# NAIST-Archlab/vsim

Hardware: AMD Instinct MI355X
Metric: decode tokens/sec GPT-J-6B Q4_0 @1 GPU; achieved HBM GB/s vs peak (higher is better)
Workload: dtype f32 (Q4_0 x Q4_0 operands); 1 GPU; gpt-j-6B Q4_0 decode, 874 timed tokens after a 5-token prompt + 5 warm-up tokens, batch 1; mode=exact, n_ctx=980, parallelism=single, graph=True

## Files before the change

include/vsim_hip.h:

```cpp
#ifndef VSIM_HIP_H
#define VSIM_HIP_H

#include <stddef.h>
#include <stdint.h>

#include "ggml_abi.h"

#ifdef __cplusplus
extern "C" {
#endif

#define VSIM_OK 0
#define VSIM_EINVAL (-1)
#define VSIM_EHIP (-2)
#define VSIM_ENOMEM (-3)
#define VSIM_EFILE (-4)
#define VSIM_ENODEV (-5)
#define VSIM_ESPIN (-6)

#define VSIM_MODE_EXACT 0
#define VSIM_MODE_FAST 1

#define VSIM_ARCH_GPTNEOX 0
#define VSIM_ARCH_GPTJ 1
// ... 47 lines not shown
int vsim_batch_set_gemm(int enable);
int vsim_op_q4_gemm_fast_rows(const void *w, int M, int K, const void *xq, int n, const float *bias, float *y,
                              void *stream);
int vsim_batch_set_fast_gemm(int enable);
typedef struct {
  const float *q, *k, *v;
  float *const *kc;
  float *const *vc;
  const int32_t *n_past;
  const double *cs;
  const float *alibi;
  int32_t B, d, H, n_rot, style, n_ctx, kqv_nth;
  float scale;
  float *out;
  void *oq;
  float *oxd;
} vsim_attn_batch_args;
int vsim_op_attn_decode_batch(const vsim_attn_batch_args *a, void *stream);
int vsim_op_q4_expand_f16(const void *w, int M, int K, void *w16, void *stream);
int vsim_op_gemm_f16(const void *w16, int M, int K, const void *x16, int n, const float *bias, float *y,
                     void *stream);
int vsim_op_act_quant_f16(const float *x, int K, int n, const float *bias, int gelu, void *x16, void *stream);
int vsim_op_gemm_f16_gelu_q(const void *w16, int M, int K, const void *x16, int n, const float *bias, void *q16,
                            void *stream);
int vsim_op_gemm_f16_rope(const void *w16, int M, int K, const void *x16, int n, const float *bias, float *y,
                          const double *cs, int d, int n_rot, int p0, void *stream);
int vsim_op_gemm_f16_join(const void *w16, int M, int K, const void *x16, int n, const float *bias, float *res,
                          const float *res_a, void *stream);
int vsim_op_gemm_q4_256(const void *w, int M, int K, const void *x16, int n, const float *bias, float *y, void *q16,
                        const double *cs, int d, int n_rot, int p0, int join, const float *res_a, void *stream);
int vsim_op_get_rows(const void *w, int K, int V, const int32_t *rows, int n, float *y, void *stream);
int vsim_op_norm(const float *x, float *y, int k, int rows, const float *w, const float *b, void *stream);
int vsim_norm_fallbacks(unsigned out[2]);
int vsim_spin_timeouts(unsigned *out);
int vsim_op_gelu(const float *x, float *y, int n, void *stream);
int vsim_op_argmax(const float *x, int n, int32_t *out, void *stream);
#define VSIM_TOPK_MAX 64
#define VSIM_WINDOW_MAX 1024
int vsim_op_topk(const float *x, int n, const int32_t *win, int nw, double scale, double repeat_penalty, int k,
                 double *val, int32_t *id, void *stream);
int vsim_op_logprob(const float *x, int V, int R, const int32_t *target, double *logprob, int32_t *argmax,
                    void *stream);
int vsim_op_attn_softmax(float *p, int nc, int nr, int nz, int n_past, float scale, void *stream);
int vsim_op_rope(int style, float *x, int d, int H, int T, int n_past, int n_dims, int mode, void *stream);
int vsim_op_kq(const float *K, int ldk, const float *Q, int ldq, int d, int H, int nk, int n, float *kq,
               void *stream);
int vsim_op_kqv(const float *V, int ldv, const float *S, int d, int H, int nk, int n, float *out, void *stream);
int vsim_op_kq_causal(const float *K, int ldk, const float *Q, int ldq, int d, int H, int nk, int n, int n_past,
                      float *kq, void *stream);
int vsim_op_kqv_causal(const float *V, int ldv, const float *S, int d, int H, int nk, int n, int n_past, float *out,
                       void *stream);
int vsim_op_attn_prefill(const float *Q, const float *kc, const float *vc, int d, int H, int N, int n_past,
                         float scale, float *out, void *stream);
int vsim_op_attn_prefill_q16(const float *Q, const float *kc, const float *vc, int d, int H, int N, int n_past,
                             float scale, void *out16, void *stream);
int vsim_gemm_set_streamk(int enable);
int vsim_op_gemm_q4_256_pair(const void *w0, const void *w1, int M, int K, const void *x16, int n, float *y0, float *y1,
                             const double *cs, int d, int n_rot, int p0, void *stream);
int vsim_gemm_set_qk_pair(int mode);
int vsim_gemm_set_tile_order(int cols);
int vsim_op_norm_f16q(const float *x, int k, int rows, const float *w, const float *b, void *x16, void *stream);
#define VSIM_FAST_PAD 65536
enum { VSIM_FE_STORE = 0, VSIM_FE_GELU_Q = 1, VSIM_FE_ROPE_Q = 2, VSIM_FE_ROPE_K = 3, VSIM_FE_V = 4 };
typedef struct {
  const void *w;
  int32_t rows, k;
// ... 116 lines not shown
```

vsim_amd/csrc/capi.cpp:

```cpp
#include <hip/hip_runtime.h>

#include <cstdio>
#include <cstdlib>
#include <cstring>
#include <mutex>
#include <unordered_map>
#include <map>
#include <vector>

#include "common.hpp"
#include "fast.hpp"
#include "graph.hpp"
#include "../../include/vsim_hip.h"

namespace vsim {
int tables_host(uint16_t *exp_f16, uint16_t *gelu_f16);
}

using namespace vsim;

#define RC(x)                \
  do {                       \
    int rc_ = (x);           \
    if (rc_) return rc_;     \
// ... 117 lines not shown
  if (!w16 || !x16 || !res) { set_error("gemm_f16_join: null argument"); return VSIM_EINVAL; }
  G2Epi e;
  e.res = res;
  e.res_a = res_a;
  return launch_gemm_f16_256(w16, M, K, x16, n, bias, res, (hipStream_t)stream, nullptr, &e);
}
int vsim_op_gemm_q4_256(const void *w, int M, int K, const void *x16, int n, const float *bias, float *y, void *q16,
                        const double *cs, int d, int n_rot, int p0, int join, const float *res_a, void *stream) {
  if (!w || !x16 || (!q16 && !y) || M <= 0 || K <= 0 || K % QK || p0 < 0) {
    set_error("gemm_q4_256: bad argument");
    return VSIM_EINVAL;
  }
  if ((q16 != nullptr) + (cs != nullptr) + (join != 0) > 1) {
    set_error("gemm_q4_256: one epilogue at a time (q16, cs or join)");
    return VSIM_EINVAL;
  }
  G2Epi e;
  if (cs) {
    e.cs = (const double2 *)cs;
    e.d = d;
    e.n_rot = n_rot;
    e.p0 = p0;
  } else if (join) {
    e.res = y;
    e.res_a = res_a;
  }
  return launch_gemm_q4_256(w4_view(w, M, K), x16, n, bias, q16 ? nullptr : y, (hipStream_t)stream, q16,
                            cs || join ? &e : nullptr);
}
int vsim_op_get_rows(const void *w, int K, int V, const int32_t *rows, int n, float *y, void *stream) {
  return launch_get_rows(w, K, V, rows, n, y, (hipStream_t)stream);
}
int vsim_norm_fallbacks(unsigned out[2]) { return vsim::norm_stats(out); }
int vsim_spin_timeouts(unsigned *out) { return vsim::spin_timeouts(out); }

int vsim_op_norm(const float *x, float *y, int k, int rows, const float *w, const float *b, void *stream) {
  return launch_norm(x, y, k, rows, w, b, (hipStream_t)stream);
}
int vsim_op_gelu(const float *x, float *y, int n, void *stream) {
  return launch_gelu(x, y, n, nullptr, 1, (hipStream_t)stream);
}
int vsim_op_argmax(const float *x, int n, int32_t *out, void *stream) {
  static std::mutex mu;
  static std::map<std::pair<int, void *>, unsigned long long *> wss;
  int dev = 0;
  VSIM_HIP(hipGetDevice(&dev));
  unsigned long long *ws = nullptr;
  {
    std::lock_guard<std::mutex> lk(mu);
    unsigned long long *&w = wss[{dev, stream}];
    if (!w) {
      VSIM_HIP(hipMalloc((void **)&w, 2 * sizeof(unsigned long long)));
      VSIM_HIP(hipMemset(w, 0, 2 * sizeof(unsigned long long)));
    }
    ws = w;
  }
  return launch_argmax(x, n, (int *)out, ws, (hipStream_t)stream);
}
int vsim_op_topk(const float *x, int n, const int32_t *win, int nw, double scale, double repeat_penalty, int k,
                 double *val, int32_t *id, void *stream) {
  static std::mutex mu;
  static std::map<std::pair<int, void *>, void *> wss;
  int dev = 0;
  VSIM_HIP(hipGetDevice(&dev));
  void *ws = nullptr;
  {
// ... 471 lines not shown
```

vsim_amd/csrc/common.hpp:

```cpp
#pragma once

#include <hip/hip_runtime.h>
#include <stdint.h>

#include <map>
#include <string>

#include "../../include/vsim_hip.h"

namespace vsim {

constexpr int QK = 32;
constexpr int QBYTES = 20;

constexpr int T32 = 32;

typedef float f32x4 __attribute__((ext_vector_type(4)));
typedef unsigned int u32x4 __attribute__((ext_vector_type(4)));

struct W4 {
  const uint8_t *qs;
  const float *d;
  int rows, k, tiles;
  __host__ __device__ int nb() const { return k / QK; }
// ... 32 lines not shown
struct GemvBatch {
  GemvJob j[4];
  int nj;
};

struct LnQuantJob {
  const float *x;
  const float *w, *b;
  uint8_t *qs;
  float *d;
  float *xd;
  const float *ja, *jab, *jf, *jfb;
  float *jout;
  unsigned *ep;
};

struct TailLn {
  const float *x;
  const float *ab, *fb;
  float *jout;
  const float *w1, *b1;
  uint8_t *q1;
  float *d1, *xd1;
  const float *w2, *b2;
  uint8_t *q2;
  float *d2, *xd2;
  unsigned long long *og, *jg;
  uint4 *rec;
  const unsigned *ep;
  unsigned *stats;
  int il;
};
constexpr int LNT_MAX_TILES = 256;

struct AttnJob {
  const float *q, *k, *v;
  float *kc, *vc;
  const int *npast;
  const double2 *cs;
  const uint16_t *etab;
  int d, H, n_rot, style;
  int n_ctx;
  int nsplit;
  int kqv_nth;
  float scale;
  const float *alibi;
  uint8_t *oq_qs;
  float *oq_d, *oxd;
  float *out;
};

constexpr int ATT_VTF = 8192;
__host__ __device__ constexpr int attn_lds_floats(int d, int n_ctx) {
  return ((2 * d + n_ctx + 3) & ~3) + 2 * ATT_VTF;
}

int launch_ln_quant(const LnQuantJob &j0, const LnQuantJob *j1, int n, hipStream_t s);
int launch_residual_join(const float *x, const float *a, const float *ab, const float *f, const float *fb, float *out,
                         int n, hipStream_t s);
int launch_gemv_epi(const GemvBatch &B, int mode, hipStream_t s);
int launch_attn_decode(const AttnJob &A, int n_ctx, hipStream_t s);
struct AttnRows {
  float *const *kc, *const *vc;
  size_t loff;
  const int *npast;
};
// ... 77 lines not shown
}

__device__ __forceinline__ float wave_sum_f(float v) {
  return dpp::lane63(dpp::reduce(v, 0.0f, [](float a, float b) { return a + b; }));
}
__device__ __forceinline__ double wave_sum_d(double v) {
  return dpp::lane63(dpp::reduce(v, 0.0, [](double a, double b) { return a + b; }));
}
__device__ __forceinline__ float wave_max_f(float v) {
  return dpp::lane63(dpp::reduce(v, -INFINITY, [](float a, float b) { return fmaxf(a, b); }));
}
__device__ __forceinline__ int wave_min_i(int v) {
  return dpp::lane63(dpp::reduce(v, 0x7FFFFFFF, [](int a, int b) { return min(a, b); }));
}

void set_error(const std::string &msg);
int hip_fail(hipError_t e, const char *what);
#define VSIM_HIP(call)                                          \
  do {                                                          \
    hipError_t e_ = (call);                                     \
    if (e_ != hipSuccess) return ::vsim::hip_fail(e_, #call);   \
  } while (0)

struct DevTables {
  const uint16_t *exp_f16;
  const uint16_t *gelu_f16;
};
int tables_get(DevTables *t);
unsigned *dev_stats();
unsigned *spin_error_counter();
unsigned *set_spin_error_target(unsigned *p);
void add_model_spin_timeouts(unsigned n);
int norm_stats(unsigned *out2);
int spin_timeouts(unsigned *out);

int launch_q4_repack(const void *aos, void *soa, int rows, int k, hipStream_t s);
int launch_q4_unpack(const void *soa, void *aos, int rows, int k, hipStream_t s);
int launch_q4_quantize(const float *x, int k, int n, void *xq, float *xd, hipStream_t s);
int launch_quantize_w(const void *x, int src_type, int rows, int k, void *w, int w_rows, int row0, void *aos,
                      uint64_t *hist, hipStream_t s);
int launch_q4_gemv(const void *w, int M, int K, const void *xq, const float *xd, int n, const float *bias,
                   float *y, int mode, hipStream_t s);
int launch_gemv_batch(const GemvBatch &B, int mode, hipStream_t s);
int launch_gemm_exact(const W4 &W, const float *xd, int n, const float *bias, float *y, hipStream_t s);
int launch_gemm_exact_rows(const W4 &W, const float *xd, int n, const float *bias, float *y, hipStream_t s);
int launch_gemm_fast_rows(const W4 &W, const void *xq, int n, const float *bias, float *y, hipStream_t s);
int batch_set_fast_gemm(int enable);
bool batch_fast_gemm_rows(int n);
int launch_act_repack(const void *aos, void *xq, int n, int k, hipStream_t s);
int launch_act_unpack(const void *xq, void *aos, int n, int k, hipStream_t s);
int launch_q4_dequant(const void *xq, int rows, int k, float *y, hipStream_t s);
int launch_get_rows(const void *w, int K, int V, const int32_t *rows, int n, float *y, hipStream_t s);
int launch_norm(const float *x, float *y, int k, int rows, const float *w, const float *b, hipStream_t s);
int launch_norm_f16q(const float *x, void *x16, int k, int rows, const float *w, const float *b, hipStream_t s);
int launch_argmax(const float *x, int n, int *out, unsigned long long *ws, hipStream_t s);
struct TopkParams {
  double scale, penalty;
  int32_t k, nw;
  int32_t win[VSIM_WINDOW_MAX];
};
struct TopkOut {
  double val[VSIM_TOPK_MAX];
  int32_t id[VSIM_TOPK_MAX];
};
constexpr int TOPK_MAX_WG = 64;
constexpr size_t TOPK_WS_BYTES = 256 + (size_t)TOPK_MAX_WG * 64 * (sizeof(unsigned long long) + sizeof(uint32_t));
// ... 79 lines not shown
```

vsim_amd/csrc/gemv_chain.hip:

```cpp
#include <cstdlib>
#include <cstring>

#ifdef VSIM_NB_STAMPS
namespace vsim {
__device__ unsigned long long g_nb_stamps[2048][32];
}
#define ATT_STAMP(i) \
  if (threadIdx.x == 0) g_nb_stamps[1536 + blockIdx.x][4 + (i)] = __builtin_amdgcn_s_memrealtime()
#endif
#include "attn.hpp"
#include "kern.hpp"
#include "../../include/vsim_hip.h"

namespace vsim {

typedef const __attribute__((address_space(4))) float sfloat;
typedef const __attribute__((address_space(1))) u32x4 gu32x4;
typedef const __attribute__((address_space(1))) float gfloat;

__device__ __forceinline__ void producer_barrier() { asm volatile("s_barrier" ::: "memory"); }


constexpr int waitcnt_vm(int n) { return 0x0F70 | (n & 15) | ((n >> 4) << 14); }
constexpr int c2_waves(int npw, bool fill) {
// ... 211 lines not shown
#define NB_ADDS4P(acc, a, o)                                                                                     \
  asm volatile(NB_PAIR(1, 2, 3, 4) NB_PAIR(5, 6, 7, 8) NB_PAIR(9, 10, 11, 12) NB_PAIR(13, 14, 15, 16)              \
               : "+v"(acc)                                                                                       \
               : "v"(a[o].x), "v"(a[o].y), "v"(a[o].z), "v"(a[o].w), "v"(a[o + 1].x), "v"(a[o + 1].y),           \
                 "v"(a[o + 1].z), "v"(a[o + 1].w), "v"(a[o + 2].x), "v"(a[o + 2].y), "v"(a[o + 2].z),            \
                 "v"(a[o + 2].w), "v"(a[o + 3].x), "v"(a[o + 3].y), "v"(a[o + 3].z), "v"(a[o + 3].w)             \
               : "memory")
#ifdef VSIM_NB_STAMPS
#define NBS(...) __VA_ARGS__
#else
#define NBS(...)
#endif
#ifndef NB_RING_N
#define NB_RING_N 4
#endif
constexpr int NB_RING = NB_RING_N;
constexpr unsigned NB_SPIN_MAX = 1u << 24;
template <class S>
struct NbLds {
  float P[NB_RING][32 * S::LD];
  uint4 RQ[S::DEPTH][S::NPW][64];
  float RD[S::DEPTH][S::NPW][64];
  float RX[S::DEPTH][S::NPW][64];
  unsigned ready[NB_RING];
  unsigned cons;
};

__device__ __forceinline__ unsigned lds_load(const unsigned *p) {
  return __hip_atomic_load(p, __ATOMIC_RELAXED, __HIP_MEMORY_SCOPE_WORKGROUP);
}

constexpr unsigned LNT_SPIN_MAX = 1u << 22;
typedef __attribute__((address_space(1))) unsigned long long gu64;
__device__ __forceinline__ unsigned lnt_tag(const TailLn &N) { return (*N.ep << 8) | (unsigned)(N.il + 1); }
__device__ __forceinline__ void st_granule(unsigned long long *p, float v, unsigned tag) {
  const unsigned long long g = (unsigned long long)__float_as_uint(v) | ((unsigned long long)tag << 32);
  __hip_atomic_store((gu64 *)p, g, __ATOMIC_RELAXED, __HIP_MEMORY_SCOPE_AGENT);
}
__device__ __forceinline__ unsigned long long ld_granule(const unsigned long long *p) {
  return __hip_atomic_load((const gu64 *)p, __ATOMIC_RELAXED, __HIP_MEMORY_SCOPE_AGENT);
}
__device__ __forceinline__ void st16_sc1(uint4 *p, u32x4 v) {
  asm volatile("global_store_dwordx4 %0, %1, off sc1" ::"v"(p), "v"(v) : "memory");
}
__device__ __forceinline__ double dbl_of(unsigned lo, unsigned hi) {
  return __longlong_as_double((long long)(((unsigned long long)hi << 32) | lo));
}
__device__ __forceinline__ void lnt_spin(unsigned &spins, unsigned *err, int lane) {
  __builtin_amdgcn_s_sleep(1);
  if (++spins == LNT_SPIN_MAX && err && lane == 0) __hip_atomic_fetch_add(err, 1u, __ATOMIC_RELAXED, __HIP_MEMORY_SCOPE_AGENT);
}

__device__ __forceinline__ void lnt_oproj(const TailLn &N, int row, int rows, float acc, int lane) {
  if (lane < 32 && row < rows) st_granule(N.og + row, acc, lnt_tag(N));
  NBS(if (lane == 0) g_nb_stamps[1536 + blockIdx.x][8] = __builtin_amdgcn_s_memrealtime();)
}

struct LntPre {
  unsigned long long g;
  float x, ab, fb, w, b;
};
__device__ __forceinline__ LntPre lnt_prefetch(const TailLn &N, int t) {
  const int lane = threadIdx.x & 63, i = t * T32 + (lane & 31);
  const bool hi = lane >= 32, mine = !hi || N.w2 != nullptr;
  LntPre p;
  p.g = ld_granule(N.og + i);
  p.x = N.x[i];
  p.ab = N.ab ? N.ab[i] : 0.0f;
  p.fb = N.fb ? N.fb[i] : 0.0f;
  p.w = mine ? (hi ? N.w2 : N.w1)[i] : 0.0f;
  p.b = mine ? (hi ? N.b2 : N.b1)[i] : 0.0f;
  return p;
}
__device__ __forceinline__ double half_sum_d(double v) {
  v = v + dpp::mov<dpp::QP_XOR1, 0xF>(v, 0.0);
  v = v + dpp::mov<dpp::QP_XOR2, 0xF>(v, 0.0);
  v = v + dpp::mov<dpp::HALF_MIRROR, 0xF>(v, 0.0);
  v = v + dpp::mov<dpp::MIRROR, 0xF>(v, 0.0);
  const long long b = __double_as_longlong(v);
  const int lo = __builtin_amdgcn_ds_swizzle((int)(b & 0xFFFFFFFF), 0x401F), hi = __builtin_amdgcn_ds_swizzle((int)(b >> 32), 0x401F);
  return v + __longlong_as_double(((long long)hi << 32) | (unsigned)lo);
}
__device__ __forceinline__ int half_min_i(int v) {
  v = min(v, dpp::mov<dpp::QP_XOR1, 0xF>(v, 0x7FFFFFFF));
  v = min(v, dpp::mov<dpp::QP_XOR2, 0xF>(v, 0x7FFFFFFF));
  v = min(v, dpp::mov<dpp::HALF_MIRROR, 0xF>(v, 0x7FFFFFFF));
  v = min(v, dpp::mov<dpp::MIRROR, 0xF>(v, 0x7FFFFFFF));
  return min(v, __builtin_amdgcn_ds_swizzle(v, 0x401F));
}

__device__ __forceinline__ void lnt_owner(const TailLn &N, int t, int ntile, float acc, const LntPre &pre,
                                          float *scr, unsigned *err) {
  const int lane = threadIdx.x & 63, i = t * T32 + (lane & 31), n = ntile * T32;
  const unsigned tag = lnt_tag(N);
  NBS(unsigned long long *ls = g_nb_stamps[1536 + blockIdx.x] + 8;
      if (lane == 0) ls[0] = __builtin_amdgcn_s_memrealtime();)
  const bool hi = lane >= 32, two = N.w2 != nullptr, mine = !hi || two;
  const float xv = pre.x, abv = pre.ab, fbv = pre.fb, wv = pre.w, bv = pre.b;
  unsigned spins = 0;
  unsigned long long ga = pre.g;
  while (!__all((unsigned)(ga >> 32) == tag) && spins < LNT_SPIN_MAX) {
    lnt_spin(spins, err, lane);
    ga = ld_granule(N.og + i);
  }
  NBS(if (lane == 0) {
    ls[1] = __builtin_amdgcn_s_memrealtime();
    ls[5] = spins;
  })
  const float a = N.ab ? __uint_as_float((unsigned)ga) + abv : __uint_as_float((unsigned)ga);
  const float ff = N.fb ? acc + fbv : acc;
  const float v = xv + (a + ff);
  {
    const double s = half_sum_d((double)v), sa = half_sum_d((double)fabsf(v));
    const double q = half_sum_d((double)v * (double)v);
    const int um = half_min_i(ulp_exp(v));
    if (lane == 0) {
      float au = (float)sa;
      if ((double)au < sa) au = __uint_as_float(__float_as_uint(au) + 1u);
      const unsigned long long sb = (unsigned long long)__double_as_longlong(s), qb = (unsigned long long)__double_as_longlong(q);
      st16_sc1(N.rec + 2 * t, u32x4{(unsigned)sb, (unsigned)(sb >> 32), (unsigned)um, tag});
      st16_sc1(N.rec + 2 * t + 1, u32x4{(unsigned)qb, (unsigned)(qb >> 32), __float_as_uint(au), tag});
    }
  }
  if (lane < 32) {
    N.jout[i] = v;
    st_granule(N.jg + i, v, tag);
  }
  NBS(if (lane == 0) ls[2] = __builtin_amdgcn_s_memrealtime();)
  const int ng = 2 * ntile;
  double S = 0.0, Q = 0.0, A = 0.0;
  int U = 1 << 30;
  spins = 0;
  for (;;) {
    u32x4 g[8];
    const uint4 *p[8];
#pragma unroll
    for (int k = 0; k < 8; ++k) p[k] = N.rec + min(lane + 64 * k, ng - 1);
    asm volatile(
        "global_load_dwordx4 %0, %8, off sc1\n\t"
        "global_load_dwordx4 %1, %9, off sc1\n\t"
        "global_load_dwordx4 %2, %10, off sc1\n\t"
        "global_load_dwordx4 %3, %11, off sc1\n\t"
        "global_load_dwordx4 %4, %12, off sc1\n\t"
        "global_load_dwordx4 %5, %13, off sc1\n\t"
        "global_load_dwordx4 %6, %14, off sc1\n\t"
        "global_load_dwordx4 %7, %15, off sc1\n\t"
        "s_waitcnt vmcnt(0)"
        : "=&v"(g[0]), "=&v"(g[1]), "=&v"(g[2]), "=&v"(g[3]), "=&v"(g[4]), "=&v"(g[5]), "=&v"(g[6]), "=&v"(g[7])
        : "v"(p[0]), "v"(p[1]), "v"(p[2]), "v"(p[3]), "v"(p[4]), "v"(p[5]), "v"(p[6]), "v"(p[7])
        : "memory");
    bool ok = true;
#pragma unroll
    for (int k = 0; k < 8; ++k)
      if (lane + 64 * k < ng) ok = ok && g[k].w == tag;
    if (__all(ok) || spins >= LNT_SPIN_MAX) {
#pragma unroll
      for (int k = 0; k < 8; ++k) {
        if (lane + 64 * k >= ng) continue;
        if ((lane & 1) == 0) {
          S += dbl_of(g[k].x, g[k].y);
          U = min(U, (int)g[k].z);
        } else {
          Q += dbl_of(g[k].x, g[k].y);
          A += (double)__uint_as_float(g[k].z);
        }
      }
      break;
    }
    lnt_spin(spins, err, lane);
  }
  NBS(if (lane == 0) {
    ls[3] = __builtin_amdgcn_s_memrealtime();
    ls[6] = spins;
  })
  S = wave_sum_d(S);
  Q = wave_sum_d(Q);
  A = wave_sum_d(A);
  U = wave_min_i(U);
  const double eps = 1e-5f;
  double mean = 0.0;
  float scale = 0.0f;
  const bool mean_ok = U == (1 << 30) || A * (1.0 + 0x1.0p-30) < ldexp(1.0, 53 + U);
  bool fallback = !mean_ok;
  if (mean_ok) {
    mean = S / n;
    const double t1 = mean * S, t3 = (mean * mean) * n;
    const double s2 = (Q - 2.0 * t1) + t3, M = Q + 2.0 * fabs(t1) + t3;
    const double s2c = s2 > 0.0 ? s2 : 0.0;
    const double B = ((2.0 * n + 64.0) * s2c + 64.0 * M) * 0x1.0p-53 * (1.0 + 0x1.0p-20);
    const double r = 1.0 / sqrt(s2 / n + eps);
    const double dr = r * (B / ((s2c - B > 0.0 ? s2c - B : 0.0) + n * eps) + 0x1.0p-48);
    const float sc = (float)r;
    if ((float)(r - dr) == sc && (float)(r + dr) == sc)
      scale = sc;
    else
      fallback = true;
  }
  if (fallback) {
    for (int k = lane; k < n; k += 64) {
      unsigned sp = 0;
      unsigned long long g;
      do {
        g = ld_granule(N.jg + k);
        if ((unsigned)(g >> 32) == tag) break;
        __builtin_amdgcn_s_sleep(1);
      } while (++sp < LNT_SPIN_MAX);
      scr[k] = __uint_as_float((unsigned)g);
    }
    __builtin_amdgcn_wave_barrier();
    asm volatile("s_waitcnt lgkmcnt(0)" ::: "memory");
    const double m = mean_ok ? S : seq_sum_exact_inl(scr, n, lane);
    mean = m / n;
    double s2 = 0.0;
    for (int k = lane; k < n; k += 64) {
      const double d = (double)scr[k] - mean;
      s2 += d * d;
    }
    s2 = wave_sum_d(s2);
    const double B = (2.0 * n + 64.0) * 0x1.0p-53 * s2;
    const float sc_lo = (float)(1.0 / sqrt((s2 + B) / n + eps));
    const float sc_hi = (float)(1.0 / sqrt((s2 - B > 0.0 ? s2 - B : 0.0) / n + eps));
    scale = sc_lo;
    if (sc_lo != sc_hi) {
      float sq = 0.0f;
      if (lane == 0) {
        double qq = 0.0;
        for (int k = 0; k < n; ++k) {
          const double d = (double)scr[k] - mean;
          qq += d * d;
        }
        sq = (float)(1.0 / sqrt(qq / n + eps));
      }
      scale = __shfl(sq, 0);
      if (t == 0 && lane == 0 && N.stats) atomicAdd(&N.stats[1], 1u);
    }
    if (!mean_ok && t == 0 && lane == 0 && N.stats) atomicAdd(&N.stats[0], 1u);
  }
  float y = (float)((double)v - mean);
  y = y * scale;
  const float z = mine ? (wv * y) + bv : 0.0f;
  uint8_t *qs = hi ? N.q2 : N.q1;
  float *dq = hi ? N.d2 : N.d1, *xd = hi ? N.xd2 : N.xd1;
  quantize_half(z, lane, mine, mine ? qs + (size_t)t * 16 : nullptr, mine ? dq + t : nullptr,
                mine ? xd + (size_t)t * QK : nullptr);
  NBS(if (lane == 0) ls[4] = __builtin_amdgcn_s_memrealtime();)
}

template <class S, bool SC1, bool ONE = false, int LNR = 0>
__device__ __forceinline__ void chain32_nb_body(const GemvBatch &B, int t, NbLds<S> &L, unsigned *err,
                                                const TailLn *N = nullptr) {
  constexpr int DEPTH = S::DEPTH, CB = S::CB, LD = S::LD, NPW = S::NPW;
  constexpr int WAIT_VM = waitcnt_vm(3 * (DEPTH - 1));
  static_assert(3 * (DEPTH - 1) < 64, "vmcnt immediate");
  const int wave = __builtin_amdgcn_readfirstlane(threadIdx.x >> 6);
  const int lane = threadIdx.x & 63;
  int ji = 0;
  if constexpr (ONE) {
    if (t >= B.j[0].w.tiles) return;
  } else {
    while (ji < B.nj) {
      if (t < B.j[ji].w.tiles) break;
      t -= B.j[ji].w.tiles;
      ++ji;
    }
    if (ji >= B.nj) return;
    ji = __builtin_amdgcn_readfirstlane(ji);
  }
  const GemvJob &J = B.j[ONE ? 0 : ji];
  const int nb = J.w.k / QK, nch = (nb + CB - 1) / CB;
// ... 90 lines not shown
  }

  float acc = 0.0f;
  const int lr = lane >> 1, lk = lane & 1;
  constexpr int NV = S::CP / 8, BQ = 4, NBQ = NV / BQ;
  static_assert(NV % BQ == 0 && NBQ % 4 == 0, "batches tile the chunk in whole rounds of four sets");
  auto need = [](int c) { return (unsigned)(NPW * (c / NB_RING + 1)); };
  NBS(unsigned long long cw = 0;)
  auto wait_ready = [&](int c, unsigned have) {
    NBS(const unsigned long long t0 = __builtin_amdgcn_s_memtime();)
    if (have < need(c)) {
      unsigned spins = 0, h;
      asm volatile(
          "1:\n\t"
          "ds_read_b32 %0, %2\n\t"
          "s_waitcnt lgkmcnt(0)\n\t"
          "v_cmp_lt_u32 vcc, %0, %3\n\t"
          "s_cbranch_vccz 2f\n\t"
          "s_add_u32 %1, %1, 1\n\t"
          "s_cmp_lt_u32 %1, %4\n\t"
          "s_cbranch_scc1 1b\n\t"
          "2:"
          : "=&v"(h), "+s"(spins)
          : "v"(lds_addr(&L.ready[c % NB_RING])), "s"(need(c)), "s"(NB_SPIN_MAX)
          : "vcc", "scc", "memory");
      if (spins >= NB_SPIN_MAX && err && lane == 0) __hip_atomic_fetch_add(err, 1u, __ATOMIC_RELAXED, __HIP_MEMORY_SCOPE_AGENT);
    }
    NBS(const unsigned long long dw = __builtin_amdgcn_s_memtime() - t0; cw += dw;
        if (ONE && blockIdx.x < 128 && c < 32 && lane == 0) {
          g_nb_stamps[960 + blockIdx.x][c] = dw;
          g_nb_stamps[1088 + blockIdx.x][c] = t0;
        })
  };
  __builtin_amdgcn_s_setprio(3);
  NBS(const unsigned long long c_t0 = __builtin_amdgcn_s_memtime();)
  wait_ready(0, 0u);
  NBS(if (ONE && LNR == 1 && lane == 0) g_nb_stamps[1536 + blockIdx.x][3] = __builtin_amdgcn_s_memrealtime();)
  f32x4 b0[BQ], b1[BQ], b2[BQ], b3[BQ];
  auto rd = [&](f32x4 (&d)[BQ], int c, int q) {
    const f32x4 *src = (const f32x4 *)&L.P[c % NB_RING][lr * LD] + 2 * q * BQ + lk;
#pragma unroll
    for (int j = 0; j < BQ; ++j) d[j] = src[2 * j];
  };
  rd(b0, 0, 0);
  rd(b1, 0, 1);
  rd(b2, 0, 2);
  LntPre pre{};
  const int c_pre = nch > 1 ? nch - 2 : 0;
  for (int c = 0; c < nch; ++c) {
    if constexpr (LNR == 1)
      if (c == c_pre) pre = lnt_prefetch(*N, t);
    unsigned rdy = 0;
#pragma unroll
    for (int q = 0; q < NBQ; ++q) {
      const int qn = q + 3, cn = qn < NBQ ? c : c + 1, qr = qn < NBQ ? qn : qn - NBQ;
      if (q == NBQ - 5) rdy = lds_load(&L.ready[(c + 1) % NB_RING]);
      if (qn == NBQ && c + 1 < nch) {
        unsigned r = rdy;
        asm volatile("" : "+v"(r));
        wait_ready(c + 1, r);
      }
      asm volatile("" ::: "memory");
      f32x4(&dst)[BQ] = (qn % 4 == 0) ? b0 : (qn % 4 == 1) ? b1 : (qn % 4 == 2) ? b2 : b3;
      rd(dst, cn, qr);
      f32x4(&cur)[BQ] = (q % 4 == 0) ? b0 : (q % 4 == 1) ? b1 : (q % 4 == 2) ? b2 : b3;
      NB_ADDS4P(acc, cur, 0);
      if (q == NBQ - 1)
        __hip_atomic_store(&L.cons, (unsigned)(c + 1), __ATOMIC_RELAXED, __HIP_MEMORY_SCOPE_WORKGROUP);
    }
  }
  __builtin_amdgcn_s_setprio(0);
  NBS(if (lane == 0) {
    g_nb_stamps[blockIdx.x][0] = c_t0;
    g_nb_stamps[blockIdx.x][1] = __builtin_amdgcn_s_memtime();
    g_nb_stamps[blockIdx.x][2] = cw;
    g_nb_stamps[blockIdx.x][3] = nch;
  })
  acc = __shfl(acc, (2 * lane) & 63);

  const int row = t * T32 + (lane & 31);
  const int rows = J.w.rows;
  const float *bias = J.bias;
  float *y = J.y;
  if constexpr (LNR == 1) {
    lnt_owner(*N, t, J.w.tiles, acc, pre, &L.P[0][0], err);
    return;
  }
  if constexpr (LNR == 2) {
    lnt_oproj(*N, row, rows, acc, lane);
    return;
  }
  if (J.epi == EPI_GELU_Q) {
    const bool ok = lane < 32 && row < rows;
    float g = 0.0f;
    if (ok) {
      g = h2f(J.gelu_tab[f2h(acc + bias[row])]);
      if (y) y[row] = g;
    }
    quantize_half(g, lane, ok, J.oq_qs + (size_t)t * 16, J.oq_d + t, J.oxd + (size_t)t * QK);
  } else if (lane < 32 && row < rows) {
    y[row] = bias ? acc + bias[row] : acc;
  }
}

constexpr unsigned TAIL_SPIN_MAX = 1u << 22;
struct TailJob {
  GemvBatch f, o;
  AttnJob a;
  TailSync sy;
  unsigned *err;
  int nf;
  int lnon;
  TailLn ln;
};

__global__ void __launch_bounds__(C2Tail::THREADS, 1) k_layer_tail(TailJob T) {
  __shared__ union {
    NbLds<C2Tail> n;
    float a[sizeof(NbLds<C2Tail>) / sizeof(float)];
  } L;
  int b = blockIdx.x;
  asm volatile("" ::"s"(T.nf), "s"(T.f.j[0].w.qs), "s"(T.f.j[0].w.d), "s"(T.f.j[0].w.k), "s"(T.f.j[0].w.tiles),
// ... 335 lines not shown
```

vsim_amd/csrc/ops_elt.hip:

```cpp
#include <cmath>
#include <cstring>
#include <atomic>
#include <mutex>
#include <vector>

#include "kern.hpp"
#include "../../include/vsim_hip.h"

namespace vsim {

__global__ void __launch_bounds__(NORM_THREADS) k_norm_exact(const float *__restrict__ X, float *__restrict__ Y, int n,
                                                              const float *__restrict__ gw,
                                                              const float *__restrict__ gb, unsigned *stats) {
  extern __shared__ __attribute__((aligned(16))) float xrow[];
  ln_exact_lds(X + (size_t)blockIdx.x * n, xrow, n, gw, gb, stats);
  float *y = Y + (size_t)blockIdx.x * n;
  for (int i = threadIdx.x; i < n; i += NORM_THREADS) y[i] = xrow[i];
}

constexpr int NORMQ_THREADS = 512;
__global__ void __launch_bounds__(NORMQ_THREADS) k_norm_f16q(const float *__restrict__ X, _Float16 *__restrict__ Q16,
                                                             int n, const float *__restrict__ gw,
                                                             const float *__restrict__ gb, unsigned *stats) {
  extern __shared__ __attribute__((aligned(16))) float xrow[];
// ... 123 lines not shown
}

static std::mutex g_tab_mu;
static std::vector<uint16_t> g_exp_host, g_gelu_host;
static DevTables g_dev_tab[64];
static bool g_dev_tab_ok[64];

static void build_host_tables() {
  if (!g_exp_host.empty()) return;
  g_exp_host.resize(65536);
  g_gelu_host.resize(65536);
  for (int i = 0; i < 65536; ++i) {
    const float f = host_h2f((uint16_t)i);
    g_gelu_host[i] = host_f2h(host_gelu(f));
    g_exp_host[i] = host_f2h((float)exp((double)f));
  }
}

int tables_get(DevTables *t) {
  int dev = 0;
  VSIM_HIP(hipGetDevice(&dev));
  std::lock_guard<std::mutex> lk(g_tab_mu);
  if (dev < 0 || dev >= 64) { set_error("tables: device id out of range"); return VSIM_EINVAL; }
  if (!g_dev_tab_ok[dev]) {
    build_host_tables();
    uint16_t *p = nullptr;
    VSIM_HIP(hipMalloc(&p, 2 * 65536 * sizeof(uint16_t)));
    VSIM_HIP(hipMemcpy(p, g_exp_host.data(), 65536 * 2, hipMemcpyHostToDevice));
    VSIM_HIP(hipMemcpy(p + 65536, g_gelu_host.data(), 65536 * 2, hipMemcpyHostToDevice));
    g_dev_tab[dev].exp_f16 = p;
    g_dev_tab[dev].gelu_f16 = p + 65536;
    g_dev_tab_ok[dev] = true;
    if (!g_dev_stats[dev]) {
      VSIM_HIP(hipMalloc(&g_dev_stats[dev], 4 * sizeof(unsigned)));
      VSIM_HIP(hipMemset(g_dev_stats[dev], 0, 4 * sizeof(unsigned)));
    }
  }
  *t = g_dev_tab[dev];
  return VSIM_OK;
}

int tables_host(uint16_t *exp_f16, uint16_t *gelu_f16) {
  std::lock_guard<std::mutex> lk(g_tab_mu);
  build_host_tables();
  memcpy(exp_f16, g_exp_host.data(), 65536 * 2);
  memcpy(gelu_f16, g_gelu_host.data(), 65536 * 2);
  return VSIM_OK;
}

static thread_local unsigned *t_err_target = nullptr;
static std::atomic<unsigned> g_model_spins{0};
unsigned *set_spin_error_target(unsigned *p) {
  unsigned *o = t_err_target;
  t_err_target = p;
  return o;
}
void add_model_spin_timeouts(unsigned n) { g_model_spins += n; }
unsigned *spin_error_counter() {
  if (t_err_target) return t_err_target;
  unsigned *st = dev_stats();
  return st ? st + 2 : nullptr;
}

static int stats_sum(int k, unsigned *out) {
  *out = 0;
  int cur = 0;
  VSIM_HIP(hipGetDevice(&cur));
  for (int dev = 0; dev < 64; ++dev) {
    if (!g_dev_stats[dev]) continue;
    unsigned v = 0;
    VSIM_HIP(hipSetDevice(dev));
    VSIM_HIP(hipMemcpy(&v, g_dev_stats[dev] + k, sizeof(unsigned), hipMemcpyDeviceToHost));
    *out += v;
  }
  VSIM_HIP(hipSetDevice(cur));
  return VSIM_OK;
}
int spin_timeouts(unsigned *out) {
  const int rc = stats_sum(2, out);
  *out += g_model_spins.load();
  return rc;
}

int norm_stats(unsigned *out2) {
  const int rc = stats_sum(0, &out2[0]);
  if (rc != VSIM_OK) return rc;
  return stats_sum(1, &out2[1]);
}

constexpr int AM_T = 256, AM_MAX_WG = 64;
static int am_grid(const float *x, int n) {
  const int n4 = ((uintptr_t)x & 15) ? 0 : n / 4;
  const int per = n4 > n - 4 * n4 ? n4 : n - 4 * n4;
  const int g = (per + AM_T - 1) / AM_T;
  return g < 1 ? 1 : g > AM_MAX_WG ? AM_MAX_WG : g;
}
template <bool GEN>
__global__ void __launch_bounds__(AM_T) k_argmax(const float *__restrict__ x, int n, int *__restrict__ out,
                                                 unsigned long long *ws, int *tok, int *npast, int *hist) {
  __shared__ unsigned long long sk[AM_T / 64];
  unsigned long long best = 0;
  const int n4 = ((uintptr_t)x & 15) ? 0 : n / 4;
  const int gt = blockIdx.x * AM_T + threadIdx.x, nt = gridDim.x * AM_T;
  const float4 *x4 = (const float4 *)x;
  for (int i = gt; i < n4; i += nt) {
    const float4 v = x4[i];
    best = max(best, am_key(v.x, 4 * i));
    best = max(best, am_key(v.y, 4 * i + 1));
    best = max(best, am_key(v.z, 4 * i + 2));
    best = max(best, am_key(v.w, 4 * i + 3));
  }
  for (int i = 4 * n4 + gt; i < n; i += nt) best = max(best, am_key(x[i], i));
#pragma unroll
  for (int o = 32; o > 0; o >>= 1) best = max(best, (unsigned long long)__shfl_xor(best, o, 64));
  if ((threadIdx.x & 63) == 0) sk[threadIdx.x >> 6] = best;
  __syncthreads();
  if (threadIdx.x != 0) return;
#pragma unroll
  for (int w = 1; w < AM_T / 64; ++w) best = max(best, sk[w]);
  unsigned *cnt = (unsigned *)(ws + 1);
// ... 33 lines not shown
```

vsim_amd/hip.py:

```python
from __future__ import annotations

import ctypes
import os

import numpy as np

HERE = os.path.dirname(os.path.abspath(__file__))
LIB_PATH = os.environ.get("VSIM_LIB") or os.path.join(HERE, "_build", "libvsim_hip.so")

MODE_EXACT = 0
MODE_FAST = 1
ARCH_GPTNEOX = 0
ARCH_GPTJ = 1
ARCH_BLOOM = 2

EXPORTS = [
    "vsim_last_error", "vsim_device_count", "vsim_q4_bytes",
    "init_xmax", "imax_ggml_compute_forward_mul_mat_q4_0_f32",
    "vsim_ggml_gptneox_rope_f32", "vsim_ggml_rope_f32", "vsim_ggml_soft_max_f32", "vsim_ggml_mul_mat_f32",
    "vsim_dropin_stats", "vsim_dropin_reset", "vsim_norm_fallbacks", "vsim_spin_timeouts",
    "vsim_op_q4_repack", "vsim_op_q4_unpack", "vsim_op_act_repack", "vsim_op_act_unpack",
    "vsim_op_q4_quantize", "vsim_op_q4_gemv", "vsim_op_q4_expand_f16", "vsim_op_gemm_f16",
    "vsim_op_act_quant_f16", "vsim_op_gemm_f16_gelu_q", "vsim_op_gemm_f16_rope", "vsim_op_gemm_f16_join",
    "vsim_op_gemm_q4_256", "vsim_op_get_rows",
    "vsim_op_norm", "vsim_op_gelu", "vsim_op_argmax", "vsim_op_attn_softmax", "vsim_op_rope", "vsim_op_kq", "vsim_op_kqv", "vsim_op_kq_causal", "vsim_op_kqv_causal",
    "vsim_op_attn_prefill", "vsim_op_attn_prefill_q16", "vsim_gemm_set_streamk", "vsim_gemm_set_qk_pair", "vsim_gemm_set_tile_order", "vsim_op_gemm_q4_256_pair", "vsim_op_norm_f16q",
    "vsim_op_tables", "vsim_op_fast_gemv", "vsim_op_fast_tail", "vsim_op_fast_oproj_join",
    "vsim_model_create", "vsim_model_load_file", "vsim_model_set_tensor", "vsim_model_get_tensor",
    "vsim_model_randomize",
    "vsim_model_set_mode", "vsim_model_reserve", "vsim_model_hparams", "vsim_model_eval", "vsim_model_eval_argmax", "vsim_model_generate",
    "vsim_model_stream",
    "vsim_model_logits_dev", "vsim_model_info", "vsim_model_set_graph", "vsim_model_set_profile",
    "vsim_model_profile_kernel", "vsim_model_profile_stats", "vsim_model_free",
    "vsim_graph_compute", "vsim_graph_compute_rc", "vsim_graph_sync_tensor", "vsim_graph_reset", "vsim_graph_stats",
    "vsim_graph_set_profile", "vsim_graph_profile_report", "vsim_graph_match", "vsim_graph_fast_stats",
    "vsim_model_stage_bind", "vsim_model_stage_begin", "vsim_model_stage_step", "vsim_model_sync",
    "vsim_model_debug_poison",
    "vsim_op_topk", "vsim_sampler_create", "vsim_sampler_accept", "vsim_sampler_pick", "vsim_sampler_sample_host",
    "vsim_sampler_stats", "vsim_sampler_free", "vsim_model_eval_sample", "vsim_model_generate_sampled",
    "vsim_op_q4_quantize_w", "vsim_model_load_file_ex", "vsim_model_set_tensor_src", "vsim_quantize_set_chunk_rows",
    "vsim_quantize_file", "vsim_quantize_set_verbose",
    "vsim_op_logprob", "vsim_model_eval_score", "vsim_score_set_chunk_rows",
    "vsim_op_q4_gemm_rows", "vsim_batch_set_gemm", "vsim_op_attn_decode_batch",
    "vsim_model_seq_reserve", "vsim_model_eval_seq", "vsim_model_decode_batch",
    "vsim_op_q4_gemm_fast_rows", "vsim_batch_set_fast_gemm", "vsim_model_decode_batch_fast",
]

BATCH_MAX = 32

SRC_F32, SRC_F16 = 0, 1
LOAD_QUANTIZE = 1

TOPK_MAX = 64
# ... 500 lines not shown
        check(lib().vsim_model_stage_bind(self.h, tok_in or None, resid_in or None, resid_out or None,
                                          tok_out or None), "stage_bind")

    def stage_begin(self, n_past: int):
        check(lib().vsim_model_stage_begin(self.h, n_past), "stage_begin")

    def stage_step(self):
        check(lib().vsim_model_stage_step(self.h), "stage_step")

    def sync(self):
        check(lib().vsim_model_sync(self.h), "sync")

    def debug_poison(self, n_tokens: int):
        check(lib().vsim_model_debug_poison(self.h, n_tokens), "debug_poison")

    def close(self):
        if getattr(self, "h", None):
            lib().vsim_model_free(self.h)
            self.h = None

    def __del__(self):
        try:
            self.close()
        except Exception:
            pass


def norm_fallbacks():
    out = (ctypes.c_uint * 2)()
    check(lib().vsim_norm_fallbacks(out), "norm_fallbacks")
    return int(out[0]), int(out[1])


def spin_timeouts():
    out = ctypes.c_uint()
    check(lib().vsim_spin_timeouts(ctypes.byref(out)), "spin_timeouts")
    return int(out.value)


def dropin_stats():
    v = [ctypes.c_uint64() for _ in range(4)]
    lib().vsim_dropin_stats(*[ctypes.byref(x) for x in v])
    return {"calls": v[0].value, "h2d": v[1].value, "d2h": v[2].value, "cached": v[3].value}
```

Before: 521.3 tokens/s.

## Add prefix-sum certificate to avoid slow fallback in fused tail layernorm

When the per-row exactness bound for the layernorm mean fails, the tail kernel now tries a wave-level prefix-sum certificate over the already-loaded partial records before dropping to the full readback fallback. The fallback readback is rewritten to batch sixteen granule loads per lane with inline asm before spinning on late tags. The tag computation is hoisted to a scalar register once per kernel. New device counters track how often each path is taken, which adds a few atomics and extra register pressure from keeping the record array live.

```diff
diff --git a/include/vsim_hip.h b/include/vsim_hip.h
--- a/include/vsim_hip.h
+++ b/include/vsim_hip.h
@@ -103,6 +103,7 @@
 int vsim_op_get_rows(const void *w, int K, int V, const int32_t *rows, int n, float *y, void *stream);
 int vsim_op_norm(const float *x, float *y, int k, int rows, const float *w, const float *b, void *stream);
 int vsim_norm_fallbacks(unsigned out[2]);
+int vsim_tail_ln_stats(unsigned out[4]);
 int vsim_spin_timeouts(unsigned *out);
 int vsim_op_gelu(const float *x, float *y, int n, void *stream);
 int vsim_op_argmax(const float *x, int n, int32_t *out, void *stream);
diff --git a/vsim_amd/csrc/capi.cpp b/vsim_amd/csrc/capi.cpp
--- a/vsim_amd/csrc/capi.cpp
+++ b/vsim_amd/csrc/capi.cpp
@@ -173,6 +173,7 @@
   return launch_get_rows(w, K, V, rows, n, y, (hipStream_t)stream);
 }
 int vsim_norm_fallbacks(unsigned out[2]) { return vsim::norm_stats(out); }
+int vsim_tail_ln_stats(unsigned out[4]) { return vsim::tail_ln_stats(out); }
 int vsim_spin_timeouts(unsigned *out) { return vsim::spin_timeouts(out); }
 
 int vsim_op_norm(const float *x, float *y, int k, int rows, const float *w, const float *b, void *stream) {
diff --git a/vsim_amd/csrc/common.hpp b/vsim_amd/csrc/common.hpp
--- a/vsim_amd/csrc/common.hpp
+++ b/vsim_amd/csrc/common.hpp
@@ -88,6 +88,7 @@
   int il;
 };
 constexpr int LNT_MAX_TILES = 256;
+constexpr int DEV_STATS_N = 8, LNT_STAT = 4;
 
 struct AttnJob {
   const float *q, *k, *v;
@@ -231,6 +232,7 @@
 unsigned *set_spin_error_target(unsigned *p);
 void add_model_spin_timeouts(unsigned n);
 int norm_stats(unsigned *out2);
+int tail_ln_stats(unsigned *out4);
 int spin_timeouts(unsigned *out);
 
 int launch_q4_repack(const void *aos, void *soa, int rows, int k, hipStream_t s);
diff --git a/vsim_amd/csrc/gemv_chain.hip b/vsim_amd/csrc/gemv_chain.hip
--- a/vsim_amd/csrc/gemv_chain.hip
+++ b/vsim_amd/csrc/gemv_chain.hip
@@ -267,7 +267,11 @@
 
 constexpr unsigned LNT_SPIN_MAX = 1u << 22;
 typedef __attribute__((address_space(1))) unsigned long long gu64;
-__device__ __forceinline__ unsigned lnt_tag(const TailLn &N) { return (*N.ep << 8) | (unsigned)(N.il + 1); }
+__device__ __forceinline__ unsigned lnt_tag(const TailLn &N) {
+  unsigned tag = __builtin_amdgcn_readfirstlane((int)((*N.ep << 8) | (unsigned)(N.il + 1)));
+  asm volatile("" : "+s"(tag));
+  return tag;
+}
 __device__ __forceinline__ void st_granule(unsigned long long *p, float v, unsigned tag) {
   const unsigned long long g = (unsigned long long)__float_as_uint(v) | ((unsigned long long)tag << 32);
   __hip_atomic_store((gu64 *)p, g, __ATOMIC_RELAXED, __HIP_MEMORY_SCOPE_AGENT);
@@ -286,8 +290,8 @@
   if (++spins == LNT_SPIN_MAX && err && lane == 0) __hip_atomic_fetch_add(err, 1u, __ATOMIC_RELAXED, __HIP_MEMORY_SCOPE_AGENT);
 }
 
-__device__ __forceinline__ void lnt_oproj(const TailLn &N, int row, int rows, float acc, int lane) {
-  if (lane < 32 && row < rows) st_granule(N.og + row, acc, lnt_tag(N));
+__device__ __forceinline__ void lnt_oproj(const TailLn &N, unsigned tag, int row, int rows, float acc, int lane) {
+  if (lane < 32 && row < rows) st_granule(N.og + row, acc, tag);
   NBS(if (lane == 0) g_nb_stamps[1536 + blockIdx.x][8] = __builtin_amdgcn_s_memrealtime();)
 }
 
@@ -324,10 +328,93 @@
   return min(v, __builtin_amdgcn_ds_swizzle(v, 0x401F));
 }
 
-__device__ __forceinline__ void lnt_owner(const TailLn &N, int t, int ntile, float acc, const LntPre &pre,
+__device__ __forceinline__ bool lnt_prefix_cert(const u32x4 (&g)[8], int ng, int G, int lane, double &total) {
+  const double lim = ldexp(1.0, 53 + G);
+  const bool ev = (lane & 1) == 0;
+  bool ok = true;
+  double base = 0.0;
+#pragma unroll
+  for (int k = 0; k < 8; ++k) {
+    if (64 * k >= ng) break;
+    const bool in = ev && lane + 64 * k < ng;
+    const double at = (double)__shfl_down(__uint_as_float(g[k].z), 1);
+    double x = in ? dbl_of(g[k].x, g[k].y) : 0.0;
+#pragma unroll
+    for (int d = 1; d < 64; d <<= 1) {
+      const double u = __shfl_up(x, d, 64);
+      if (lane >= d) x += u;
+      ok = ok && fabs(x) < lim;
+    }
+    double ex = __shfl_up(x, 1, 64);
+    if (lane == 0) ex = 0.0;
+    const double p = base + ex;
+    ok = ok && fabs(p) < lim;
+    if (in) ok = ok && (fabs(p) + at) * (1.0 + 0x1.0p-30) < lim;
+    base = base + rl_d(x, 63);
+    ok = ok && fabs(base) < lim;
+  }
+  total = base;
+  return __all(ok);
+}
+
+__device__ __forceinline__ void lnt_readback(const unsigned long long *jg, int n, unsigned tag, float *scr,
+                                             unsigned *err, int lane) {
+  unsigned spins = 0;
+  for (int c = 0; c < n; c += 64 * 16) {
+    const int k0 = c + lane;
+    unsigned long long a[8], b[8];
+    const unsigned long long *pa[8], *pb[8];
+#pragma unroll
+    for (int j = 0; j < 8; ++j) {
+      pa[j] = jg + min(k0 + 64 * j, n - 1);
+      pb[j] = jg + min(k0 + 64 * (j + 8), n - 1);
+    }
+    asm volatile(
+        "global_load_dwordx2 %0, %8, off sc1\n\t"
+        "global_load_dwordx2 %1, %9, off sc1\n\t"
+        "global_load_dwordx2 %2, %10, off sc1\n\t"
+        "global_load_dwordx2 %3, %11, off sc1\n\t"
+        "global_load_dwordx2 %4, %12, off sc1\n\t"
+        "global_load_dwordx2 %5, %13, off sc1\n\t"
+        "global_load_dwordx2 %6, %14, off sc1\n\t"
+        "global_load_dwordx2 %7, %15, off sc1"
+        : "=&v"(a[0]), "=&v"(a[1]), "=&v"(a[2]), "=&v"(a[3]), "=&v"(a[4]), "=&v"(a[5]), "=&v"(a[6]), "=&v"(a[7])
+        : "v"(pa[0]), "v"(pa[1]), "v"(pa[2]), "v"(pa[3]), "v"(pa[4]), "v"(pa[5]), "v"(pa[6]), "v"(pa[7])
+        : "memory");
+    asm volatile(
+        "global_load_dwordx2 %0, %16, off sc1\n\t"
+        "global_load_dwordx2 %1, %17, off sc1\n\t"
+        "global_load_dwordx2 %2, %18, off sc1\n\t"
+        "global_load_dwordx2 %3, %19, off sc1\n\t"
+        "global_load_dwordx2 %4, %20, off sc1\n\t"
+        "global_load_dwordx2 %5, %21, off sc1\n\t"
+        "global_load_dwordx2 %6, %22, off sc1\n\t"
+        "global_load_dwordx2 %7, %23, off sc1\n\t"
+        "s_waitcnt vmcnt(0)"
+        : "=&v"(b[0]), "=&v"(b[1]), "=&v"(b[2]), "=&v"(b[3]), "=&v"(b[4]), "=&v"(b[5]), "=&v"(b[6]), "=&v"(b[7]),
+          "+v"(a[0]), "+v"(a[1]), "+v"(a[2]), "+v"(a[3]), "+v"(a[4]), "+v"(a[5]), "+v"(a[6]), "+v"(a[7])
+        : "v"(pb[0]), "v"(pb[1]), "v"(pb[2]), "v"(pb[3]), "v"(pb[4]), "v"(pb[5]), "v"(pb[6]), "v"(pb[7])
+        : "memory");
+#pragma unroll
+    for (int j = 0; j < 16; ++j) {
+      const int k = k0 + 64 * j;
+      unsigned long long v = j < 8 ? a[j] : b[j - 8];
+      bool late = k < n && (unsigned)(v >> 32) != tag;
+      while (__any(late) && spins < LNT_SPIN_MAX) {
+        lnt_spin(spins, err, lane);
+        if (late) {
+          v = ld_granule(jg + k);
+          late = (unsigned)(v >> 32) != tag;
+        }
+      }
+      if (k < n) scr[k] = __uint_as_float((unsigned)v);
+    }
+  }
+}
+
+__device__ __forceinline__ void lnt_owner(const TailLn &N, unsigned tag, int t, int ntile, float acc, const LntPre &pre,
                                           float *scr, unsigned *err) {
   const int lane = threadIdx.x & 63, i = t * T32 + (lane & 31), n = ntile * T32;
-  const unsigned tag = lnt_tag(N);
   NBS(unsigned long long *ls = g_nb_stamps[1536 + blockIdx.x] + 8;
       if (lane == 0) ls[0] = __builtin_amdgcn_s_memrealtime();)
   const bool hi = lane >= 32, two = N.w2 != nullptr, mine = !hi || two;
@@ -366,8 +453,8 @@
   double S = 0.0, Q = 0.0, A = 0.0;
   int U = 1 << 30;
   spins = 0;
+  u32x4 g[8];
   for (;;) {
-    u32x4 g[8];
     const uint4 *p[8];
 #pragma unroll
     for (int k = 0; k < 8; ++k) p[k] = N.rec + min(lane + 64 * k, ng - 1);
@@ -415,7 +502,14 @@
   const double eps = 1e-5f;
   double mean = 0.0;
   float scale = 0.0f;
-  const bool mean_ok = U == (1 << 30) || A * (1.0 + 0x1.0p-30) < ldexp(1.0, 53 + U);
+  const bool row_ok = U == (1 << 30) || A * (1.0 + 0x1.0p-30) < ldexp(1.0, 53 + U);
+  bool pfx_ok = false;
+  if (!row_ok) {
+    double tot = 0.0;
+    pfx_ok = lnt_prefix_cert(g, ng, U, lane, tot);
+    if (pfx_ok) S = tot;
+  }
+  const bool mean_ok = row_ok || pfx_ok;
   bool fallback = !mean_ok;
   if (mean_ok) {
     mean = S / n;
@@ -432,16 +526,7 @@
       fallback = true;
   }
   if (fallback) {
-    for (int k = lane; k < n; k += 64) {
-      unsigned sp = 0;
-      unsigned long long g;
-      do {
-        g = ld_granule(N.jg + k);
-        if ((unsigned)(g >> 32) == tag) break;
-        __builtin_amdgcn_s_sleep(1);
-      } while (++sp < LNT_SPIN_MAX);
-      scr[k] = __uint_as_float((unsigned)g);
-    }
+    lnt_readback(N.jg, n, tag, scr, err, lane);
     __builtin_amdgcn_wave_barrier();
     asm volatile("s_waitcnt lgkmcnt(0)" ::: "memory");
     const double m = mean_ok ? S : seq_sum_exact_inl(scr, n, lane);
@@ -467,9 +552,17 @@
         sq = (float)(1.0 / sqrt(qq / n + eps));
       }
       scale = __shfl(sq, 0);
-      if (t == 0 && lane == 0 && N.stats) atomicAdd(&N.stats[1], 1u);
-    }
-    if (!mean_ok && t == 0 && lane == 0 && N.stats) atomicAdd(&N.stats[0], 1u);
+      if (t == 0 && lane == 0 && N.stats) {
+        atomicAdd(&N.stats[1], 1u);
+        atomicAdd(&N.stats[LNT_STAT + 3], 1u);
+      }
+    }
+    if (t == 0 && lane == 0 && N.stats) atomicAdd(&N.stats[LNT_STAT + 2], 1u);
+  }
+  if (!row_ok && t == 0 && lane == 0 && N.stats) {
+    atomicAdd(&N.stats[0], 1u);
+    atomicAdd(&N.stats[LNT_STAT], 1u);
+    if (pfx_ok) atomicAdd(&N.stats[LNT_STAT + 1], 1u);
   }
   float y = (float)((double)v - mean);
   y = y * scale;
@@ -626,6 +719,9 @@
           g_nb_stamps[1088 + blockIdx.x][c] = t0;
         })
   };
+  unsigned lnt = 0;
+  if constexpr (LNR != 0) lnt = lnt_tag(*N);
+  (void)lnt;
   __builtin_amdgcn_s_setprio(3);
   NBS(const unsigned long long c_t0 = __builtin_amdgcn_s_memtime();)
   wait_ready(0, 0u);
@@ -677,11 +773,11 @@
   const float *bias = J.bias;
   float *y = J.y;
   if constexpr (LNR == 1) {
-    lnt_owner(*N, t, J.w.tiles, acc, pre, &L.P[0][0], err);
+    lnt_owner(*N, lnt, t, J.w.tiles, acc, pre, &L.P[0][0], err);
     return;
   }
   if constexpr (LNR == 2) {
-    lnt_oproj(*N, row, rows, acc, lane);
+    lnt_oproj(*N, lnt, row, rows, acc, lane);
     return;
   }
   if (J.epi == EPI_GELU_Q) {
diff --git a/vsim_amd/csrc/ops_elt.hip b/vsim_amd/csrc/ops_elt.hip
--- a/vsim_amd/csrc/ops_elt.hip
+++ b/vsim_amd/csrc/ops_elt.hip
@@ -179,8 +179,8 @@
     g_dev_tab[dev].gelu_f16 = p + 65536;
     g_dev_tab_ok[dev] = true;
     if (!g_dev_stats[dev]) {
-      VSIM_HIP(hipMalloc(&g_dev_stats[dev], 4 * sizeof(unsigned)));
-      VSIM_HIP(hipMemset(g_dev_stats[dev], 0, 4 * sizeof(unsigned)));
+      VSIM_HIP(hipMalloc(&g_dev_stats[dev], DEV_STATS_N * sizeof(unsigned)));
+      VSIM_HIP(hipMemset(g_dev_stats[dev], 0, DEV_STATS_N * sizeof(unsigned)));
     }
   }
   *t = g_dev_tab[dev];
@@ -233,6 +233,14 @@
   const int rc = stats_sum(0, &out2[0]);
   if (rc != VSIM_OK) return rc;
   return stats_sum(1, &out2[1]);
+}
+
+int tail_ln_stats(unsigned *out4) {
+  for (int k = 0; k < 4; ++k) {
+    const int rc = stats_sum(LNT_STAT + k, &out4[k]);
+    if (rc != VSIM_OK) return rc;
+  }
+  return VSIM_OK;
 }
 
 constexpr int AM_T = 256, AM_MAX_WG = 64;
diff --git a/vsim_amd/hip.py b/vsim_amd/hip.py
--- a/vsim_amd/hip.py
+++ b/vsim_amd/hip.py
@@ -18,7 +18,7 @@
     "vsim_last_error", "vsim_device_count", "vsim_q4_bytes",
     "init_xmax", "imax_ggml_compute_forward_mul_mat_q4_0_f32",
     "vsim_ggml_gptneox_rope_f32", "vsim_ggml_rope_f32", "vsim_ggml_soft_max_f32", "vsim_ggml_mul_mat_f32",
-    "vsim_dropin_stats", "vsim_dropin_reset", "vsim_norm_fallbacks", "vsim_spin_timeouts",
+    "vsim_dropin_stats", "vsim_dropin_reset", "vsim_norm_fallbacks", "vsim_tail_ln_stats", "vsim_spin_timeouts",
     "vsim_op_q4_repack", "vsim_op_q4_unpack", "vsim_op_act_repack", "vsim_op_act_unpack",
     "vsim_op_q4_quantize", "vsim_op_q4_gemv", "vsim_op_q4_expand_f16", "vsim_op_gemm_f16",
     "vsim_op_act_quant_f16", "vsim_op_gemm_f16_gelu_q", "vsim_op_gemm_f16_rope", "vsim_op_gemm_f16_join",
@@ -585,6 +585,12 @@
     return int(out[0]), int(out[1])
 
 
+def tail_ln_stats():
+    out = (ctypes.c_uint * 4)()
+    check(lib().vsim_tail_ln_stats(out), "tail_ln_stats")
+    return tuple(int(v) for v in out)
+
+
 def spin_timeouts():
     out = ctypes.c_uint()
     check(lib().vsim_spin_timeouts(ctypes.byref(out)), "spin_timeouts")
```

New measurement: 525.7 tokens/s, median of 6. No clear change (+0.8%).
